# lhaippp/DMHomo

Hardware: AMD Instinct MI355X
Metric: sampled images/sec (128x128, s_step=32) (higher is better)
Workload: dtype f32; 1 GPU; DGM CFG-Unet dim=64 128x128 bs=25/GPU s_step=32 cond_scale=3 (BASELINE configs[1]); global_batch=25, cfg_mode=streams, hip_graph=True, weights=seeded random init

## Files before the change

### dmhomo_amd/_lib.py

```python
import ctypes as C
import os

import torch

_HERE = os.path.dirname(os.path.abspath(__file__))
LIB_PATH = os.environ.get('DMH_LIB_PATH') or os.path.join(_HERE, 'libdmhomo_hip.so')

c_f32p = C.c_void_p
c_i64 = C.c_int64
c_int = C.c_int
c_float = C.c_float


ABI_VERSION = 500


class DmhConv(C.Structure):
    _fields_ = [('struct_size', C.c_uint64)] + \
               [(n, C.c_void_p) for n in ('src0', 'src1', 'wpack', 'bias', 'in_coef', 'res', 'res_coef', 'out',
                                          'stats')] + \
               [(n, C.c_int32) for n in ('B', 'Hin', 'Win', 'C0', 'C1', 'Cout', 'KH', 'KW', 'stride', 'upsample2')] + \
               [('in_bound', C.c_void_p), ('in_bound_n', C.c_int32), ('fin_n', C.c_int32), ('fin_w', C.c_void_p),
                ('fin_b', C.c_void_p), ('fin_out', C.c_void_p), ('pix_stats', C.c_void_p), ('pix_eps', C.c_float),
                ('rows', C.c_void_p)]
# ... 96 lines not shown
    'dmh_linear': (c_int, [c_f32p, c_i64, c_f32p, c_f32p, c_f32p, c_i64, c_int, c_int, c_int, c_int, c_int,
                           C.c_void_p]),
    'dmh_ss_gather': (c_int, [c_f32p, c_f32p, c_f32p, C.c_void_p, C.c_void_p, C.c_void_p, c_int, c_f32p, c_int, c_int, c_int,
                              C.c_void_p]),
    'dmh_assemble_input': (c_int, [c_f32p, c_int, c_f32p, c_int, c_f32p, c_f32p, c_int, c_int, c_int, c_int,
                                   C.c_void_p]),
    'dmh_final_conv_nchw': (c_int, [c_f32p, c_f32p, c_f32p, c_f32p, c_int, c_int, c_int, c_int, C.c_void_p]),
    'dmh_sampler_step': (c_int, [C.POINTER(DmhStep), c_f32p, c_f32p, c_f32p, c_f32p, c_f32p, c_f32p, c_f32p, c_i64,
                                 C.c_void_p, c_i64, C.c_void_p]),
    'dmh_sampler_step_dev': (c_int, [C.c_void_p, c_f32p, c_f32p, c_f32p, c_f32p, c_f32p, c_f32p, c_f32p, c_i64, C.c_void_p,
                                     c_i64, C.c_void_p]),
    'dmh_sampler_seek': (c_int, [C.c_void_p, c_int, C.c_void_p, C.c_void_p, c_int, C.c_void_p, C.c_void_p, c_int,
                                 C.c_void_p]),
    'dmh_sampler_step_ddp_dev': (c_int, [C.c_void_p, C.c_void_p, C.c_void_p, c_f32p, c_f32p, c_f32p, C.c_void_p, C.c_void_p,
                                         c_f32p, c_f32p, c_int, c_int, c_int, c_int, c_int, C.c_void_p]),
    'dmh_rng_indexed': (c_int, [c_f32p, c_int, c_i64, C.c_void_p, C.c_void_p, c_int, C.c_void_p]),
    'dmh_rng_keep_mask': (c_int, [C.c_void_p, c_int, C.c_void_p, C.c_void_p, c_float, C.c_void_p]),
    'dmh_rows_lincomb': (c_int, [c_f32p, c_f32p, c_f32p, c_f32p, c_f32p, c_f32p, c_int, c_i64, c_int, C.c_void_p]),
    'dmh_pixel_grid': (c_int, [c_f32p, c_int, c_int, c_int, c_float, C.c_void_p]),
    'dmh_norm_grid': (c_int, [c_f32p, c_f32p, c_int, c_int, c_int, C.c_void_p]),
    'dmh_homography_flow_points': (c_int, [C.c_void_p, C.c_void_p, C.c_void_p, c_int, c_int, c_int, c_int, c_int, C.c_void_p]),
    'dmh_dlt_points': (c_int, [C.c_void_p, C.c_void_p, C.c_void_p, C.c_void_p, c_int, c_int, C.c_void_p]),
    'dmh_affine': (c_int, [c_f32p, c_f32p, c_float, c_float, c_i64, C.c_void_p]),
    'dmh_affine_tail': (c_int, [c_f32p, c_int, c_int, c_int, c_int, c_float, c_float, C.c_void_p]),
    'dmh_q_sample': (c_int, [c_f32p, c_f32p, c_f32p, c_f32p, c_f32p, c_int, c_i64, C.c_void_p]),
    'dmh_diff_mean': (c_int, [c_f32p, c_f32p, c_f32p, c_int, C.c_void_p, c_f32p, c_int, c_int, c_int, C.c_void_p]),
    'dmh_loss_combine': (c_int, [c_f32p, c_f32p, c_f32p, c_f32p, c_int, C.c_void_p]),
    'dmh_to_uint8': (c_int, [c_f32p, C.c_void_p, c_i64, C.c_void_p]),
    'dmh_homography_flow': (c_int, [C.c_void_p, c_f32p, c_f32p, c_int, c_int, c_int, c_float, C.c_void_p]),
    'dmh_flow_to_image': (c_int, [c_f32p, c_f32p, c_int, c_int, c_float, C.c_void_p]),
# ... 55 lines not shown
```

### dmhomo_amd/cfg.py

```python
import torch
from torch import nn

from . import _params as P
from . import ops
from ._lib import DmhStep
from .engine import UnetEngine
from .sampling import DeviceRng, ModelPrediction, ScheduleHost, default, exists, extract
from .schedule import make_buffers, ddim_pairs, linear_beta_schedule, cosine_beta_schedule


class Unet(nn.Module):

    def __init__(self, dim, num_classes, cond_drop_prob=0.5, init_dim=None, out_dim=None, dim_mults=(1, 2, 4, 8),
                 channels=3, resnet_block_groups=8, learned_variance=False, learned_sinusoidal_cond=False,
                 random_fourier_features=False, learned_sinusoidal_dim=16):
        super().__init__()
        self.cond_drop_prob = cond_drop_prob
        self.channels = channels
        input_channels = channels + 3
        init_dim = default(init_dim, dim)
        self.init_conv = nn.Conv2d(input_channels, init_dim, 7, padding=3)
        time_dim = dim * 4
        self.random_or_learned_sinusoidal_cond = learned_sinusoidal_cond or random_fourier_features
        pos_emb, fourier_dim = P.time_embedding(dim, learned_sinusoidal_cond, random_fourier_features, learned_sinusoidal_dim)
# ... 25 lines not shown
        key = (int(batch), str(torch.device(device)))
        z = cache.get(key)
        if z is None:
            z = cache[key] = torch.zeros((batch,), device=device, dtype=torch.uint8)
        return z

    def _stem(self, x, rgb_flow, mask):
        if not x.is_cuda:
            raise RuntimeError('dmhomo_amd.Unet runs on the GPU only (HIP kernels); move the inputs with .cuda()')
        eng = self._engine
        eng.ensure_prepared()
        xin = ops.assemble_input(x.to(torch.float32).contiguous(), rgb_flow.to(torch.float32).contiguous(),
                                 mask.to(torch.float32).contiguous(), reps=1, cpad=eng.cin_pad)
        return eng.stem(xin)

    def _run(self, x, time, classes, rgb_flow, mask, keeps, taps=None, x0=None, first=None, out=None, rows=None):
        eng = self._engine
        if x0 is None:
            x0 = self._stem(x, rgb_flow, mask)
        if len(keeps) > 1:
            x0 = x0.repeat(len(keeps), 1, 1, 1)
        time = time.to(torch.int64).contiguous()
        classes = classes.to(torch.int64).contiguous()
        tab = self.__dict__.get('_ss_tab')
        if tab is not None:
            T, Ct, cursor = tab
            B = classes.shape[0]
            ss_all = torch.empty((len(keeps) * B, T.shape[1]), device=T.device, dtype=torch.float32)
            for r, k in enumerate(keeps):
                ops.ss_gather(T, Ct, eng.mlp_b, cursor, classes, k, out=ss_all[r * B:(r + 1) * B])
            return eng.trunk(x0, None, taps, first=first, out=out, ss_all=ss_all, rows=rows)
        cond = eng.embed(time, [(classes, k) for k in keeps], len(keeps))
        return eng.trunk(x0, cond, taps, first=first, out=out, rows=rows)

    def forward(self, x, time, classes, rgb_flow, mask, cond_drop_prob=None):
        cond_drop_prob = default(cond_drop_prob, self.cond_drop_prob)
        keep = self._keep_mask(x.shape[0], cond_drop_prob, x.device)
        return self._run(x, time, classes, rgb_flow, mask, [keep])

    cfg_mode = 'batched'
    stream_splits = 1

    def _cond_null(self, x, time, classes, rgb_flow, mask):
        B = x.shape[0]
        keep = self._keep_mask(B, self.cond_drop_prob, x.device)
        null = self._null_mask(B, x.device)
        dedup = bool(self.dedup_dropped_rows) and keep is not None
        if self.cfg_mode == 'streams':
            nsub = max(1, min(int(self.stream_splits), B))
            nstreams = 2 * nsub
            if len(getattr(self, '_side', ())) != nstreams:
                self._side = tuple(torch.cuda.Stream(device=x.device) for _ in range(nstreams))
            cur = torch.cuda.current_stream()
            x0 = self._stem(x, rgb_flow, mask)
            first = self._engine.first_conv(x0)
            cond_out = torch.empty((B, self.out_dim) + tuple(x.shape[2:]), device=x.device, dtype=torch.float32)
            null_out = torch.empty_like(cond_out)
            bounds = [(i * B) // nsub for i in range(nsub + 1)]
            si = 0
            for k, dst, sub in ((keep, cond_out, dedup), (null, null_out, False)):
                for lo, hi in zip(bounds[:-1], bounds[1:]):
                    st = self._side[si]
                    si += 1
                    st.wait_stream(cur)
                    with torch.cuda.stream(st):
                        kk = None if k is None else k[lo:hi].contiguous()
                        fs = None if first is None else (first[0][lo:hi], first[1][lo:hi])
                        self._run(None, time[lo:hi], classes[lo:hi], None, None, [kk], x0=x0[lo:hi], first=fs, out=dst[lo:hi],
                                  rows=ops.rows_from_keep(kk) if sub else None)
            for st in self._side:
                cur.wait_stream(st)
            return cond_out, null_out, (keep if dedup else None)
        both = self._run(x, time, classes, rgb_flow, mask, [keep, null],
                         rows=ops.rows_from_keep(keep, extra=B) if dedup else None)
        return both[:B], both[B:], (keep if dedup else None)

    dedup_dropped_rows = False

    def forward_with_cond_scale(self, *args, cond_scale=1., **kwargs):
        if cond_scale == 1:
            return self.forward(*args, **kwargs)
        if 'cond_drop_prob' in kwargs or len(args) > 5:
            raise TypeError("forward() got multiple values for keyword argument 'cond_drop_prob'")
        x, time, classes, rgb_flow, mask = _bind_forward(self.forward, args, kwargs)
        logits, null, computed = self._cond_null(x, time, classes, rgb_flow, mask)
        step = DmhStep(objective=ops.OBJECTIVE['pred_x0'], clip=0, mode=ops.MODE_LAST, cond_scale=float(cond_scale),
                       sqrt_recip_ac=1., sqrt_recipm1_ac=1.)
        out, _, _ = ops.sampler_step(step, logits, null, null, None, want_x_start=False, keep=computed)
        return out
# ... 113 lines not shown
        rgb_flow = ops.affine(rgb_flow.to(torch.float32), 2., -1.)
        return self.ddim_sample(classes, rgb_flow, flow, mask, shape, cond_scale)

    def _graph_tables(self, cond_scale, clip=True):
        times, steps, draws = map(list, zip(*self._ddim_steps(clip, cond_scale)))
        return steps, times, draws

    def _sample_graphed(self, classes, rgb_flow, flow, mask, shape, cond_scale):
        m, eng, device = self.model, self.model._engine, classes.device
        clip = True
        key = (tuple(shape), tuple(rgb_flow.shape), float(cond_scale), m.cfg_mode, int(m.stream_splits),
               bool(m.dedup_dropped_rows), float(m.cond_drop_prob), self.sampling_timesteps,
               self.num_timesteps, self.objective, float(self.ddim_sampling_eta), clip, self.rng.graph_key())

        def buffers(st, times, draws):
            ins = st['ins'] = [classes.clone(), rgb_flow.to(torch.float32).clone(), mask.clone()]
            st['rf'] = torch.empty_like(ins[1])
            ops.affine(ins[1], 2., -1., out=st['rf'])
            T_tab, C_tab = eng.ss_tables(times)
            st['ss_tab'] = (T_tab, C_tab, st['cursor'])

            def mid():
                cond, null, computed = self._network(st['img'], st['tcond'], ins[0], st['rf'], ins[2], cond_scale)
                noise = self.rng.randn(shape, device).contiguous()
                ops.sampler_step_dev(st['cur'], cond, null, st['img'], noise, out=st['img'], keep=computed)
                ops.sampler_seek(st['cursor'], -1, st['table'], st['times'], st['cur'], st['tcond'])

            def last():
                cond, null, computed = self._network(st['img'], st['tcond'], ins[0], st['rf'], ins[2], cond_scale)
                x0 = ops.sampler_step_dev(st['cur'], cond, null, st['img'], None, keep=computed)
                return ops.affine(x0, 0.5, 0.5)
            return mid, last

        def fill(st):
            for dst, src in zip(st['ins'], (classes, rgb_flow, mask)):
                dst.copy_(src)
            ops.affine(st['ins'][1], 2., -1., out=st['rf'])
            st['img'].copy_(self.rng.randn(shape, device))
        img = self._replay_captured(shape, device, key, lambda: self._graph_tables(cond_scale, clip), buffers, fill)
        return img, mask, flow

    @torch.no_grad()
    def interpolate(self, x1, x2, t=None, lam=0.5):
        raise TypeError('classifier_free_guidance.GaussianDiffusion.interpolate is not callable in the reference '
                        '(CFG:733 vs CFG:639); use denoising_diffusion_pytorch.GaussianDiffusion.interpolate')

    def q_sample(self, x_start, t, noise=None):
        noise = default(noise, lambda: self.rng.randn(x_start.shape, x_start.device))
        ca = self.sqrt_alphas_cumprod.gather(-1, t).contiguous()
        cb = self.sqrt_one_minus_alphas_cumprod.gather(-1, t).contiguous()
        return ops.q_sample(x_start.contiguous(), noise.contiguous(), ca, cb)

    @property
# ... 46 lines not shown
```

### dmhomo_amd/csrc/embed.hip

```cpp
#include "common.h"

__global__ void sinusoidal_embed_kernel(const int64_t* __restrict__ t, const float* __restrict__ freq,
                                        float* __restrict__ out, int R, int dim) {
  const int idx = blockIdx.x * blockDim.x + threadIdx.x;
  const int half = dim / 2;
  if (idx >= R * half) return;
  const int r = idx / half, i = idx % half;
  const float arg = (float)t[r] * freq[i];
  out[(size_t)r * dim + i] = sinf(arg);
  out[(size_t)r * dim + half + i] = cosf(arg);
}

__global__ void fourier_embed_kernel(const int64_t* __restrict__ t, const float* __restrict__ w, float* __restrict__ out, int R,
                                     int half) {
  const int idx = blockIdx.x * blockDim.x + threadIdx.x;
  if (idx >= R * half) return;
  const int r = idx / half, i = idx % half;
  const float x = (float)t[r];
  const float arg = ((x * w[i]) * 2.0f) * 3.14159265358979323846f;
  float* o = out + (size_t)r * (2 * half + 1);
  if (i == 0) o[0] = x;
  o[1 + i] = sinf(arg);
  o[1 + half + i] = cosf(arg);
}
// ... 49 lines not shown
  if (o < out_dim && r0 + ks < R) {
    const float* q = red + (ks * 4) * 64 + ol;
    float v = (q[0] + q[64]) + (q[128] + q[192]);
    if (bias) v += bias[o];
    y[(r0 + ks) * y_stride + o] = act_f(v, act_out);
  }
}

__global__ __launch_bounds__(256) void ss_gather_kernel(const float* __restrict__ T, const float* __restrict__ Ct,
                                                        const float* __restrict__ bias, const int32_t* __restrict__ cursor,
                                                        const int64_t* __restrict__ classes, const unsigned char* __restrict__ keep,
                                                        int ncls, float* __restrict__ out, int N, int S) {
  const int b = blockIdx.y;
  const int o4 = (blockIdx.x * 256 + threadIdx.x) * 4;
  if (o4 >= N) return;
  const int step = *cursor;
  const bool kept = keep ? keep[b] != 0 : true;
  const int64_t cls = classes[b];
  if ((unsigned)step >= (unsigned)S || (kept && (cls < 0 || cls >= ncls))) {
    const float q = __builtin_nanf("");
    st4(out + (size_t)b * N + o4, make_float4(q, q, q, q));
    return;
  }
  const int row = kept ? (int)cls : ncls;
  const float4 t = ld4(T + (size_t)step * N + o4), c = ld4(Ct + (size_t)row * N + o4), bb = ld4(bias + o4);
  st4(out + (size_t)b * N + o4, make_float4((t.x + c.x) + bb.x, (t.y + c.y) + bb.y, (t.z + c.z) + bb.z, (t.w + c.w) + bb.w));
}

extern "C" int dmh_ss_gather(const float* T, const float* C, const float* bias, const int32_t* cursor, const int64_t* classes,
                             const uint8_t* keep, int ncls, float* out, int B, int N, int S, void* stream) {
  DMH_REQUIRE(T && C && bias && cursor && classes && out && B > 0 && N > 0 && N % 4 == 0 && ncls > 0 && B <= 65535 && S > 0,
              "dmh_ss_gather: bad arguments");
  hipLaunchKernelGGL(ss_gather_kernel, dim3(cdiv(N / 4, 256), B), dim3(256), 0, (hipStream_t)stream, T, C, bias, cursor, classes,
                     keep, ncls, out, N, S);
  DMH_CHECK_LAUNCH("dmh_ss_gather");
  return DMH_OK;
}

extern "C" int dmh_sinusoidal_embed(const int64_t* t, const float* freq, float* out, int R, int dim, void* stream) {
  DMH_REQUIRE(t && freq && out && R > 0 && dim > 0 && dim % 2 == 0, "dmh_sinusoidal_embed: bad arguments");
  const int total = R * (dim / 2);
// ... 34 lines not shown
```

### dmhomo_amd/csrc/philox.h

```cpp
#pragma once
#include "common.h"

#pragma clang fp contract(off)

namespace dmh_philox {

struct U4 {
  uint32_t x, y, z, w;
};

__device__ __forceinline__ U4 philox4x32_10(U4 c, uint32_t k0, uint32_t k1) {
#pragma unroll
  for (int r = 0; r < 10; ++r) {
    const uint32_t hi0 = __umulhi(0xD2511F53u, c.x), lo0 = 0xD2511F53u * c.x;
    const uint32_t hi1 = __umulhi(0xCD9E8D57u, c.z), lo1 = 0xCD9E8D57u * c.z;
    c = U4{hi1 ^ c.y ^ k0, lo1, hi0 ^ c.w ^ k1, lo0};
    k0 += 0x9E3779B9u;
    k1 += 0xBB67AE85u;
  }
  return c;
}

__device__ __forceinline__ float u01(uint32_t x) { return (float)x * 2.3283064365386963e-10f + 1.1641532182693481e-10f; }

__device__ __forceinline__ void box_muller(uint32_t a, uint32_t b, float& n0, float& n1) {
  const float r = sqrtf(-2.0f * logf(u01(a)));
  float s, c;
  sincospif(2.0f * u01(b), &s, &c);
  n0 = r * c;
  n1 = r * s;
}

__device__ __forceinline__ void normal4(uint64_t seed, uint64_t draw, uint64_t sid, uint64_t q, float v[4]) {
  const U4 r = philox4x32_10(U4{(uint32_t)q, (uint32_t)draw, (uint32_t)sid, (uint32_t)(sid >> 32)}, (uint32_t)seed,
                             (uint32_t)(seed >> 32));
  box_muller(r.x, r.y, v[0], v[1]);
  box_muller(r.z, r.w, v[2], v[3]);
}

}
```

### dmhomo_amd/csrc/rng.hip

```cpp
#include "common.h"
#include "philox.h"

#pragma clang fp contract(off)

namespace {

using namespace dmh_philox;

__global__ __launch_bounds__(256) void rng_indexed_kernel(float* __restrict__ out, int64_t per, const int64_t* __restrict__ ids,
                                                          unsigned long long* state, int kind) {
  const unsigned long long seed = state[0], draw = state[1];
  const int b = blockIdx.y;
  const unsigned long long sid = (unsigned long long)ids[b];
  float* o = out + (size_t)b * per;
  const int64_t nq = (per + 3) >> 2;
  for (int64_t q = (int64_t)blockIdx.x * 256 + threadIdx.x; q < nq; q += (int64_t)gridDim.x * 256) {
    const U4 r = philox4x32_10(U4{(uint32_t)q, (uint32_t)draw, (uint32_t)sid, (uint32_t)(sid >> 32)}, (uint32_t)seed,
                               (uint32_t)(seed >> 32));
    float v[4];
    if (kind == 0) {
      box_muller(r.x, r.y, v[0], v[1]);
      box_muller(r.z, r.w, v[2], v[3]);
    } else if (kind == 1) {
      v[0] = (float)(r.x >> 8) * 5.9604644775390625e-8f;
// ... 13 lines not shown
  __syncthreads();
  if (threadIdx.x == 0) {
    const unsigned long long total = (unsigned long long)gridDim.x * gridDim.y;
    const unsigned long long t = atomicAdd(&state[2], 1ull);
    if (t == total - 1) {
      state[2] = 0;
      state[1] = draw + 1;
    }
  }
}

__global__ __launch_bounds__(256) void rng_keep_mask_kernel(unsigned char* __restrict__ keep, int B, const int64_t* __restrict__ ids,
                                                            unsigned long long* state, float prob) {
  const unsigned long long seed = state[0], draw = state[1];
  for (int b = threadIdx.x; b < B; b += 256) {
    const unsigned long long sid = (unsigned long long)ids[b];
    const U4 r = philox4x32_10(U4{0u, (uint32_t)draw, (uint32_t)sid, (uint32_t)(sid >> 32)}, (uint32_t)seed, (uint32_t)(seed >> 32));
    keep[b] = ((float)(r.x >> 8) * 5.9604644775390625e-8f) < prob ? 1 : 0;
  }
  __syncthreads();
  if (threadIdx.x == 0) state[1] = draw + 1;
}

}

extern "C" int dmh_rng_keep_mask(uint8_t* keep, int B, const int64_t* sample_ids, uint64_t* state, float prob, void* stream) {
  DMH_REQUIRE(keep && sample_ids && state && B > 0 && B <= 65535, "dmh_rng_keep_mask: bad arguments");
  hipLaunchKernelGGL(rng_keep_mask_kernel, dim3(1), dim3(256), 0, (hipStream_t)stream, keep, B, sample_ids,
                     (unsigned long long*)state, prob);
  DMH_CHECK_LAUNCH("dmh_rng_keep_mask");
  return DMH_OK;
}

// ... 16 lines not shown
```

### dmhomo_amd/csrc/sampler.hip

```cpp
#include "common.h"
#include "philox.h"

#pragma clang fp contract(off)

__global__ __launch_bounds__(256) void assemble_input_kernel(const float* __restrict__ a, int Ca,
                                                             const float* __restrict__ b, int Cb,
                                                             const float* __restrict__ m, float* __restrict__ out,
                                                             int B, int HW, int Cpad, int64_t total) {
  for (int64_t idx = (int64_t)blockIdx.x * 256 + threadIdx.x; idx < total; idx += (int64_t)gridDim.x * 256) {
    const int c = (int)(idx % Cpad);
    const int64_t rp = idx / Cpad;
    const int p = (int)(rp % HW);
    const int r = (int)(rp / HW);
    const int s = r % B;
    float v = 0.f;
    if (c < Ca) {
      v = a[((size_t)s * Ca + c) * HW + p];
    } else if (c < Ca + Cb) {
      v = b[((size_t)s * Cb + (c - Ca)) * HW + p];
      if (m) v = v * m[(size_t)s * HW + p];
    }
    out[idx] = v;
  }
}
// ... 81 lines not shown
#pragma unroll
      for (int o = 0; o < COUT; ++o) {
        const float t = row16_sum(acc[o]);
        mine = sub == o ? t : mine;
      }
      if (sub < COUT) {
        const unsigned r = (unsigned)pix / (unsigned)HW, p = (unsigned)pix - r * (unsigned)HW;
        out[((size_t)r * COUT + sub) * HW + p] = mine + bo;
      }
    }
  }
}

__device__ __forceinline__ float clamp_pm1(float x) { return x != x ? x : fminf(fmaxf(x, -1.f), 1.f); }

__global__ __launch_bounds__(256) void sampler_step_kernel(DmhStep s, const float* __restrict__ mc,
                                                           const float* __restrict__ mn, const float* __restrict__ x,
                                                           const float* __restrict__ noise, float* __restrict__ img_out,
                                                           float* __restrict__ x_start, float* __restrict__ pred_noise,
                                                           int64_t n, const uint8_t* __restrict__ keep, int64_t per_row) {
  for (int64_t i = (int64_t)blockIdx.x * 256 + threadIdx.x; i < n; i += (int64_t)gridDim.x * 256) {
    float mo;
    if (mn) {
      const float nl = mn[i];
      mo = (keep && !keep[i / per_row]) ? nl : mc[i];
      mo = nl + (mo - nl) * s.cond_scale;
    } else {
      mo = mc[i];
    }
    const float xt = x[i];
    float x0, pn;
    if (s.objective == 0) {
      pn = mo;
      x0 = s.sqrt_recip_ac * xt - s.sqrt_recipm1_ac * pn;
      if (s.clip) x0 = clamp_pm1(x0);
    } else if (s.objective == 1) {
      x0 = mo;
      if (s.clip) x0 = clamp_pm1(x0);
      pn = (s.sqrt_recip_ac * xt - x0) / s.sqrt_recipm1_ac;
    } else {
      x0 = s.sqrt_ac * xt - s.sqrt_1m_ac * mo;
      if (s.clip) x0 = clamp_pm1(x0);
      pn = (s.sqrt_recip_ac * xt - x0) / s.sqrt_recipm1_ac;
    }
    float o;
    if (s.mode == 0) {
      o = x0 * s.c0 + s.c1 * pn + s.c2 * noise[i];
    } else if (s.mode == 1) {
      o = x0;
    } else {
      o = s.c0 * x0 + s.c1 * xt;
      if (noise) o = o + s.c2 * noise[i];
    }
    img_out[i] = o;
    if (x_start) x_start[i] = x0;
    if (pred_noise) pred_noise[i] = pn;
  }
}

__global__ __launch_bounds__(256) void sampler_step_dev_kernel(const DmhStep* __restrict__ sp, const float* __restrict__ mc,
                                                               const float* __restrict__ mn, const float* x,
                                                               const float* __restrict__ noise, float* img_out,
                                                               float* __restrict__ x_start, float* __restrict__ pred_noise,
                                                               int64_t n, const uint8_t* __restrict__ keep, int64_t per_row) {
  const DmhStep s = *sp;
  for (int64_t i = (int64_t)blockIdx.x * 256 + threadIdx.x; i < n; i += (int64_t)gridDim.x * 256) {
    float mo;
    if (mn) {
      const float nl = mn[i];
      mo = (keep && !keep[i / per_row]) ? nl : mc[i];
      mo = nl + (mo - nl) * s.cond_scale;
    } else {
      mo = mc[i];
    }
    const float xt = x[i];
    float x0, pn;
    if (s.objective == 0) {
      pn = mo;
      x0 = s.sqrt_recip_ac * xt - s.sqrt_recipm1_ac * pn;
      if (s.clip) x0 = clamp_pm1(x0);
    } else if (s.objective == 1) {
      x0 = mo;
      if (s.clip) x0 = clamp_pm1(x0);
      pn = (s.sqrt_recip_ac * xt - x0) / s.sqrt_recipm1_ac;
    } else {
      x0 = s.sqrt_ac * xt - s.sqrt_1m_ac * mo;
      if (s.clip) x0 = clamp_pm1(x0);
      pn = (s.sqrt_recip_ac * xt - x0) / s.sqrt_recipm1_ac;
    }
    float o;
    if (s.mode == 0) {
      o = x0 * s.c0 + s.c1 * pn + s.c2 * (noise ? noise[i] : __builtin_nanf(""));
    } else if (s.mode == 1) {
      o = x0;
    } else {
      o = s.c0 * x0 + s.c1 * xt;
      if (noise) o = o + s.c2 * noise[i];
    }
    img_out[i] = o;
    if (x_start) x_start[i] = x0;
    if (pred_noise) pred_noise[i] = pn;
  }
}

template <int P>
__global__ __launch_bounds__(256) void sampler_step_ddp_kernel(const DmhStep* __restrict__ sp, const int32_t* __restrict__ cursor,
                                                               const int32_t* __restrict__ draws, const float* __restrict__ mc,
                                                               float* img, const float* __restrict__ noise,
                                                               const int64_t* __restrict__ ids, unsigned long long* state,
                                                               float* __restrict__ x_start, float* __restrict__ xin, int C, int HW,
                                                               int cpad, int sc, int64_t ngroups) {
  const DmhStep s = *sp;
  const bool drawn = draws[*cursor] != 0;
// ... 32 lines not shown
      } else if (drawn && noise) {
        if constexpr (P == 4) {
          const float4 n4 = ld4(noise + base);
          nz[0] = n4.x, nz[1] = n4.y, nz[2] = n4.z, nz[3] = n4.w;
        } else {
          nz[0] = noise[base];
        }
      } else {
#pragma unroll
        for (int j = 0; j < P; ++j) nz[j] = __builtin_nanf("");
      }
#pragma unroll
      for (int j = 0; j < P; ++j) {
        const float m = mo[j], x = xt[j];
        float x0, pn;
        if (s.objective == 0) {
          pn = m;
          x0 = s.sqrt_recip_ac * x - s.sqrt_recipm1_ac * pn;
          if (s.clip) x0 = clamp_pm1(x0);
        } else if (s.objective == 1) {
          x0 = m;
          if (s.clip) x0 = clamp_pm1(x0);
          pn = (s.sqrt_recip_ac * x - x0) / s.sqrt_recipm1_ac;
        } else {
          x0 = s.sqrt_ac * x - s.sqrt_1m_ac * m;
          if (s.clip) x0 = clamp_pm1(x0);
          pn = (s.sqrt_recip_ac * x - x0) / s.sqrt_recipm1_ac;
        }
        float o;
        if (s.mode == 0) {
          o = x0 * s.c0 + s.c1 * pn + s.c2 * nz[j];
        } else if (s.mode == 1) {
          o = x0;
        } else {
          o = s.c0 * x0 + s.c1 * x;
          if (drawn) o = o + s.c2 * nz[j];
        }
        img[base + j] = o;
        if (x_start) x_start[base + j] = x0;
        if (xo) {
          if (sc) {
            xo[(size_t)j * cpad + c] = x0;
            xo[(size_t)j * cpad + C + c] = o;
          } else {
            xo[(size_t)j * cpad + c] = o;
          }
        }
      }
    }
    if (xo) {
      for (int k = cin; k < cpad; ++k)
#pragma unroll
        for (int j = 0; j < P; ++j) xo[(size_t)j * cpad + k] = 0.f;
    }
  }
  if (keyed) {
    __syncthreads();
    if (threadIdx.x == 0) {
      const unsigned long long t = atomicAdd(&state[2], 1ull);
      if (t == (unsigned long long)gridDim.x - 1) {
        state[2] = 0;
        state[1] = draw + 1;
      }
    }
  }
}

__global__ __launch_bounds__(64) void sampler_seek_kernel(int32_t* cursor, int k, const DmhStep* __restrict__ table,
                                                          const int64_t* __restrict__ times, int S, DmhStep* cur,
                                                          int64_t* tcond, int B) {
  int c = k >= 0 ? k : *cursor + 1;
  c = c < S ? c : S - 1;
  __syncthreads();
  if (threadIdx.x == 0) {
    *cursor = c;
    *cur = table[c];
  }
  const int64_t t = times[c];
  for (int i = threadIdx.x; i < B; i += 64) tcond[i] = t;
// ... 175 lines not shown
                    (((uintptr_t)model_out | (uintptr_t)img | (uintptr_t)noise | (uintptr_t)x_start) & 15) == 0;
  const int64_t ngroups = (int64_t)B * HW / (quad ? 4 : 1);
  unsigned grid = grid_for(ngroups);
  grid = grid < 1024 ? grid : 1024;
  hipStream_t st = (hipStream_t)stream;
  if (quad)
    hipLaunchKernelGGL(sampler_step_ddp_kernel<4>, dim3(grid), dim3(256), 0, st, cur_dev, cursor, draws, model_out, img, noise,
                       sample_ids, (unsigned long long*)state, x_start, xin_next, C, HW, cpad, self_cond, ngroups);
  else
    hipLaunchKernelGGL(sampler_step_ddp_kernel<1>, dim3(grid), dim3(256), 0, st, cur_dev, cursor, draws, model_out, img, noise,
                       sample_ids, (unsigned long long*)state, x_start, xin_next, C, HW, cpad, self_cond, ngroups);
  DMH_CHECK_LAUNCH("dmh_sampler_step_ddp_dev");
  return DMH_OK;
}

__global__ __launch_bounds__(64) void rows_from_keep_kernel(const uint8_t* __restrict__ keep, int B, int extra,
                                                            int32_t* __restrict__ rows) {
  int n = 0;
  for (int b0 = 0; b0 < B; b0 += 64) {
    const int b = b0 + (int)threadIdx.x;
    const bool k = b < B && keep[b] != 0;
    const unsigned long long m = __ballot(k);
    if (k) rows[1 + n + __popcll(m & ((1ull << threadIdx.x) - 1ull))] = b;
    n += __popcll(m);
  }
  for (int j = threadIdx.x; j < extra; j += 64) rows[1 + n + j] = B + j;
  if (threadIdx.x == 0) rows[0] = n + extra;
}

extern "C" int dmh_rows_from_keep(const uint8_t* keep, int B, int extra, int32_t* rows, void* stream) {
// ... 76 lines not shown
```

### dmhomo_amd/ops.py

```python
import ctypes as C

import os

import torch

from . import _lib
from ._lib import call, ptr, lib

F32 = torch.float32


def _empty(shape, like, dtype=F32):
    return torch.empty(shape, device=like.device, dtype=dtype)


def ws_standardize(w, eps=1e-5):
    w = w.detach().contiguous()
    out = torch.empty_like(w)
    cout = w.shape[0]
    call('dmh_ws_standardize', ptr(w), ptr(out), cout, w.numel() // cout, float(eps))
    return out


class PackBatch:
# ... 358 lines not shown
    cin = Cc * (2 if self_cond else 1)
    if xin is not None:
        if xin.dim() != 4 or tuple(xin.shape[:3]) != (B, H, W):
            raise ValueError(f'sampler_step_ddp_dev: xin {tuple(xin.shape)} against img {(B, Cc, H, W)}')
        cpad = xin.shape[3]
    else:
        cpad = (cin + 3) // 4 * 4
    if sample_ids is not None and sample_ids.shape[0] < B:
        raise ValueError(f'sampler_step_ddp_dev: {sample_ids.shape[0]} sample ids for {B} rows')
    call('dmh_sampler_step_ddp_dev', ptr(cur, torch.uint8), ptr(cursor, torch.int32), ptr(draws, torch.int32), ptr(model_out),
         ptr(img), ptr(noise), ptr(sample_ids, torch.int64), ptr(state, torch.int64), ptr(x_start), ptr(xin), B, Cc, H * W, cpad,
         int(bool(self_cond)))
    return img


def rng_indexed(shape, sample_ids, state, kind=0):
    B = int(shape[0])
    assert sample_ids.shape == (B,) and state.shape == (4,) and state.dtype == torch.int64
    out = torch.empty(tuple(shape), device=sample_ids.device, dtype=F32)
    call('dmh_rng_indexed', ptr(out), B, out.numel() // B, ptr(sample_ids, torch.int64), ptr(state, torch.int64), int(kind))
    return out


def rng_keep_mask(sample_ids, state, prob):
    B = sample_ids.shape[0]
    out = torch.empty((B,), device=sample_ids.device, dtype=torch.uint8)
    call('dmh_rng_keep_mask', ptr(out, torch.uint8), B, ptr(sample_ids, torch.int64), ptr(state, torch.int64), float(prob))
    return out


def affine(x, scale, shift, out=None):
    x = x.contiguous()
    y = torch.empty_like(x) if out is None else out
    call('dmh_affine', ptr(x), ptr(y), float(scale), float(shift), x.numel())
    return y


def lerp(a, b, lam):
    B = a.shape[0]
    ca = torch.full((B,), 1.0 - lam, device=a.device, dtype=torch.float32)
    cb = torch.full((B,), lam, device=a.device, dtype=torch.float32)
# ... 451 lines not shown
```

### include/dmhomo_hip.h

```cpp
#ifndef DMHOMO_HIP_H
#define DMHOMO_HIP_H

#include <stdint.h>

#ifdef __cplusplus
extern "C" {
#endif

#define DMH_OK 0
#define DMH_EINVAL (-1)
#define DMH_ELAUNCH (-2)

const char* dmh_last_error(void);
#define DMH_ABI_VERSION 500
int dmh_version(void);


int dmh_ws_standardize(const float* w, float* w_out, int Cout, int K, float eps, void* stream);

int64_t dmh_conv_pack_floats(int Cout, int C0, int C1, int KH, int KW);

int dmh_pack_conv_weight(const float* w_oihw, float* wpack, int Cout, int C0, int C1, int KH, int KW,
                         void* stream);
typedef struct DmhPackJob {
// ... 108 lines not shown
} DmhStep;
int dmh_sampler_step(const DmhStep* s, const float* model_cond, const float* model_null, const float* x,
                     const float* noise, float* img_out, float* x_start, float* pred_noise, int64_t n,
                     const uint8_t* keep, int64_t per_row, void* stream);

int dmh_sampler_step_dev(const DmhStep* cur_dev, const float* model_cond, const float* model_null, const float* x,
                         const float* noise, float* img_out, float* x_start, float* pred_noise, int64_t n,
                         const uint8_t* keep, int64_t per_row, void* stream);
int dmh_sampler_seek(int32_t* cursor, int k, const DmhStep* table, const int64_t* times, int S, DmhStep* cur,
                     int64_t* tcond, int B, void* stream);

int dmh_sampler_step_ddp_dev(const DmhStep* cur_dev, const int32_t* cursor, const int32_t* draws, const float* model_out,
                             float* img, const float* noise, const int64_t* sample_ids, uint64_t* state, float* x_start,
                             float* xin_next, int B, int C, int HW, int cpad, int self_cond, void* stream);

int dmh_rng_indexed(float* out, int B, int64_t per_sample, const int64_t* sample_ids, uint64_t* state, int kind,
                    void* stream);

int dmh_rng_keep_mask(uint8_t* keep, int B, const int64_t* sample_ids, uint64_t* state, float prob, void* stream);

int dmh_affine(const float* x, float* y, float scale, float shift, int64_t n, void* stream);
int dmh_affine_tail(float* x, int B, int C, int HW, int c0, float scale, float shift, void* stream);
int dmh_rows_lincomb(const float* x, const float* y, const float* ca, const float* cb, const float* dv, float* out, int B,
                     int64_t per_sample, int clamp, void* stream);
int dmh_q_sample(const float* x_start, const float* noise, const float* ca, const float* cb, float* out, int B,
                 int64_t per_sample, void* stream);
int dmh_diff_mean(const float* a, const float* b, const float* m, int squared, double* ws, float* out, int B, int C,
                  int HW, void* stream);
int dmh_loss_combine(const float* l, const float* photo, const float* w, float* out, int B, void* stream);
int dmh_to_uint8(const float* img, uint8_t* out, int64_t n, void* stream);
// ... 79 lines not shown
```

Measured before the change: 93.10 images/s.

## Fuse CFG sampler step with next-step input assembly, keep mask and scale-shift gather

Adds a fused device kernel for the classifier-free-guidance sampling loop. In one launch it applies the guided DDIM update, writes the next step's padded NHWC network input, redraws the keep mask, gathers the cond and null scale/shift rows, and advances the cursor and step state. The network path reuses these prepared buffers instead of re-running the stem assembly and ss_gather per stream split. This removes several small kernel launches per step inside the captured graph, in exchange for a last-block atomic handoff and a more complex state protocol.

```diff
diff --git a/dmhomo_amd/_lib.py b/dmhomo_amd/_lib.py
--- a/dmhomo_amd/_lib.py
+++ b/dmhomo_amd/_lib.py
@@ -134,6 +134,10 @@
                                  C.c_void_p]),
     'dmh_sampler_step_ddp_dev': (c_int, [C.c_void_p, C.c_void_p, C.c_void_p, c_f32p, c_f32p, c_f32p, C.c_void_p, C.c_void_p,
                                          c_f32p, c_f32p, c_int, c_int, c_int, c_int, c_int, C.c_void_p]),
+    'dmh_sampler_step_cfg_dev': (c_int, [C.c_void_p, C.c_void_p, C.c_void_p, c_int, C.c_void_p, C.c_void_p, C.c_void_p, c_f32p,
+                                         c_f32p, c_f32p, c_f32p, C.c_void_p, C.c_void_p, C.c_void_p, c_float, c_int, c_int,
+                                         c_f32p, c_f32p, c_f32p, C.c_void_p, c_int, c_f32p, c_f32p, c_int, c_int, c_int, c_int,
+                                         c_int, C.c_void_p]),
     'dmh_rng_indexed': (c_int, [c_f32p, c_int, c_i64, C.c_void_p, C.c_void_p, c_int, C.c_void_p]),
     'dmh_rng_keep_mask': (c_int, [C.c_void_p, c_int, C.c_void_p, C.c_void_p, c_float, C.c_void_p]),
     'dmh_rows_lincomb': (c_int, [c_f32p, c_f32p, c_f32p, c_f32p, c_f32p, c_f32p, c_int, c_i64, c_int, C.c_void_p]),
diff --git a/dmhomo_amd/cfg.py b/dmhomo_amd/cfg.py
--- a/dmhomo_amd/cfg.py
+++ b/dmhomo_amd/cfg.py
@@ -63,17 +63,19 @@
                                  mask.to(torch.float32).contiguous(), reps=1, cpad=eng.cin_pad)
         return eng.stem(xin)
 
-    def _run(self, x, time, classes, rgb_flow, mask, keeps, taps=None, x0=None, first=None, out=None, rows=None):
+    def _run(self, x, time, classes, rgb_flow, mask, keeps, taps=None, x0=None, first=None, out=None, rows=None, ss_all=None):
         eng = self._engine
         if x0 is None:
             x0 = self._stem(x, rgb_flow, mask)
         if len(keeps) > 1:
             x0 = x0.repeat(len(keeps), 1, 1, 1)
+        if ss_all is not None:
+            return eng.trunk(x0, None, taps, first=first, out=out, ss_all=ss_all, rows=rows)
         time = time.to(torch.int64).contiguous()
         classes = classes.to(torch.int64).contiguous()
         tab = self.__dict__.get('_ss_tab')
         if tab is not None:
-            T, Ct, cursor = tab
+            T, Ct, cursor = tab[:3]
             B = classes.shape[0]
             ss_all = torch.empty((len(keeps) * B, T.shape[1]), device=T.device, dtype=torch.float32)
             for r, k in enumerate(keeps):
@@ -92,22 +94,25 @@
 
     def _cond_null(self, x, time, classes, rgb_flow, mask):
         B = x.shape[0]
-        keep = self._keep_mask(B, self.cond_drop_prob, x.device)
+        tab = self.__dict__.get('_ss_tab')
+        prep = tab[3] if tab is not None and len(tab) > 3 else None
+        keep = prep['keep'] if prep is not None else self._keep_mask(B, self.cond_drop_prob, x.device)
         null = self._null_mask(B, x.device)
         dedup = bool(self.dedup_dropped_rows) and keep is not None
+        ss = (None, None) if prep is None else (prep['ss'][:B], prep['ss'][B:])
         if self.cfg_mode == 'streams':
             nsub = max(1, min(int(self.stream_splits), B))
             nstreams = 2 * nsub
             if len(getattr(self, '_side', ())) != nstreams:
                 self._side = tuple(torch.cuda.Stream(device=x.device) for _ in range(nstreams))
             cur = torch.cuda.current_stream()
-            x0 = self._stem(x, rgb_flow, mask)
+            x0 = self._engine.stem(prep['xin']) if prep is not None else self._stem(x, rgb_flow, mask)
             first = self._engine.first_conv(x0)
             cond_out = torch.empty((B, self.out_dim) + tuple(x.shape[2:]), device=x.device, dtype=torch.float32)
             null_out = torch.empty_like(cond_out)
             bounds = [(i * B) // nsub for i in range(nsub + 1)]
             si = 0
-            for k, dst, sub in ((keep, cond_out, dedup), (null, null_out, False)):
+            for k, dst, sub, ssp in ((keep, cond_out, dedup, ss[0]), (null, null_out, False, ss[1])):
                 for lo, hi in zip(bounds[:-1], bounds[1:]):
                     st = self._side[si]
                     si += 1
@@ -116,12 +121,12 @@
                         kk = None if k is None else k[lo:hi].contiguous()
                         fs = None if first is None else (first[0][lo:hi], first[1][lo:hi])
                         self._run(None, time[lo:hi], classes[lo:hi], None, None, [kk], x0=x0[lo:hi], first=fs, out=dst[lo:hi],
-                                  rows=ops.rows_from_keep(kk) if sub else None)
+                                  rows=ops.rows_from_keep(kk) if sub else None, ss_all=None if ssp is None else ssp[lo:hi])
             for st in self._side:
                 cur.wait_stream(st)
             return cond_out, null_out, (keep if dedup else None)
-        both = self._run(x, time, classes, rgb_flow, mask, [keep, null],
-                         rows=ops.rows_from_keep(keep, extra=B) if dedup else None)
+        both = self._run(x, time, classes, rgb_flow, mask, [keep, null], x0=None if prep is None else self._engine.stem(prep['xin']),
+                         rows=ops.rows_from_keep(keep, extra=B) if dedup else None, ss_all=None if prep is None else prep['ss'])
         return both[:B], both[B:], (keep if dedup else None)
 
     dedup_dropped_rows = False
@@ -265,11 +270,13 @@
                self.num_timesteps, self.objective, float(self.ddim_sampling_eta), clip, self.rng.graph_key())
 
         def buffers(st, times, draws):
-            ins = st['ins'] = [classes.clone(), rgb_flow.to(torch.float32).clone(), mask.clone()]
+            ins = st['ins'] = [classes.to(torch.int64).clone(), rgb_flow.to(torch.float32).clone(), mask.clone()]
             st['rf'] = torch.empty_like(ins[1])
             ops.affine(ins[1], 2., -1., out=st['rf'])
             T_tab, C_tab = eng.ss_tables(times)
             st['ss_tab'] = (T_tab, C_tab, st['cursor'])
+            if fused:
+                return fused_bodies(st, draws, T_tab, C_tab)
 
             def mid():
                 cond, null, computed = self._network(st['img'], st['tcond'], ins[0], st['rf'], ins[2], cond_scale)
@@ -283,11 +290,48 @@
                 return ops.affine(x0, 0.5, 0.5)
             return mid, last
 
+        B = int(shape[0])
+        fused = self.rng.keyed and cond_scale != 1 and (shape[2] * shape[3]) % 4 == 0
+        prob = 1 - m.cond_drop_prob
+        mask_drawn = m.cond_drop_prob > 0 and 0 < prob < 1
+
+        def fused_bodies(st, draws, T_tab, C_tab):
+            ins = st['ins']
+            st['draws'] = torch.tensor(draws, dtype=torch.int32).to(device)
+            st['xin'] = torch.zeros((B, shape[2], shape[3], eng.cin_pad), device=device)
+            st['ss'] = torch.zeros((2 * B, T_tab.shape[1]), device=device)
+            st['first'] = torch.zeros((1,), dtype=torch.int32, device=device)
+            if mask_drawn:
+                st['keep'] = torch.zeros((B,), device=device, dtype=torch.uint8)
+            else:
+                st['keep'] = m._null_mask(B, device) if m.cond_drop_prob > 0 and prob == 0 else None
+            st['ids'] = self.rng.ids_for(B)
+            st['ss_tab'] = (T_tab, C_tab, st['cursor'], {'xin': st['xin'], 'keep': st['keep'], 'ss': st['ss']})
+
+            def step():
+                cond, null, computed = self._network(st['img'], st['tcond'], ins[0], st['rf'], ins[2], cond_scale)
+                ops.sampler_step_cfg_dev(st['table'], st['times'], st['draws'], st['cursor'], st['cur'], st['tcond'], cond, null,
+                                         st['img'], st['xin'], st['ids'], self.rng.state, st['keep'],
+                                         prob if mask_drawn else None, computed is not None, T_tab, C_tab, eng.mlp_b, ins[0],
+                                         st['ss'][:B], st['ss'][B:])
+
+            def last():
+                step()
+                return ops.affine(st['img'], 0.5, 0.5)
+            return step, last
+
         def fill(st):
             for dst, src in zip(st['ins'], (classes, rgb_flow, mask)):
                 dst.copy_(src)
             ops.affine(st['ins'][1], 2., -1., out=st['rf'])
             st['img'].copy_(self.rng.randn(shape, device))
+            if 'xin' in st:
+                ins, (T_tab, C_tab) = st['ins'], st['ss_tab'][:2]
+                if mask_drawn:
+                    ops.rng_keep_mask(st['ids'], self.rng.state, prob, out=st['keep'])
+                ops.assemble_input(st['img'], st['rf'], ins[2].to(torch.float32).contiguous(), cpad=eng.cin_pad, out=st['xin'])
+                ops.ss_gather(T_tab, C_tab, eng.mlp_b, st['first'], ins[0], st['keep'], out=st['ss'][:B])
+                ops.ss_gather(T_tab, C_tab, eng.mlp_b, st['first'], ins[0], m._null_mask(B, device), out=st['ss'][B:])
         img = self._replay_captured(shape, device, key, lambda: self._graph_tables(cond_scale, clip), buffers, fill)
         return img, mask, flow
 
diff --git a/dmhomo_amd/csrc/embed.hip b/dmhomo_amd/csrc/embed.hip
--- a/dmhomo_amd/csrc/embed.hip
+++ b/dmhomo_amd/csrc/embed.hip
@@ -1,4 +1,5 @@
 #include "common.h"
+#include "ss_rows.h"
 
 __global__ void sinusoidal_embed_kernel(const int64_t* __restrict__ t, const float* __restrict__ freq,
                                         float* __restrict__ out, int R, int dim) {
@@ -87,17 +88,7 @@
   const int b = blockIdx.y;
   const int o4 = (blockIdx.x * 256 + threadIdx.x) * 4;
   if (o4 >= N) return;
-  const int step = *cursor;
-  const bool kept = keep ? keep[b] != 0 : true;
-  const int64_t cls = classes[b];
-  if ((unsigned)step >= (unsigned)S || (kept && (cls < 0 || cls >= ncls))) {
-    const float q = __builtin_nanf("");
-    st4(out + (size_t)b * N + o4, make_float4(q, q, q, q));
-    return;
-  }
-  const int row = kept ? (int)cls : ncls;
-  const float4 t = ld4(T + (size_t)step * N + o4), c = ld4(Ct + (size_t)row * N + o4), bb = ld4(bias + o4);
-  st4(out + (size_t)b * N + o4, make_float4((t.x + c.x) + bb.x, (t.y + c.y) + bb.y, (t.z + c.z) + bb.z, (t.w + c.w) + bb.w));
+  ss_row_quad(T, Ct, bias, *cursor, S, keep ? keep[b] != 0 : true, classes[b], ncls, N, o4, out + (size_t)b * N);
 }
 
 extern "C" int dmh_ss_gather(const float* T, const float* C, const float* bias, const int32_t* cursor, const int64_t* classes,
diff --git a/dmhomo_amd/csrc/philox.h b/dmhomo_amd/csrc/philox.h
--- a/dmhomo_amd/csrc/philox.h
+++ b/dmhomo_amd/csrc/philox.h
@@ -38,4 +38,9 @@
   box_muller(r.z, r.w, v[2], v[3]);
 }
 
+__device__ __forceinline__ bool keep_bit(uint64_t seed, uint64_t draw, uint64_t sid, float prob) {
+  const U4 r = philox4x32_10(U4{0u, (uint32_t)draw, (uint32_t)sid, (uint32_t)(sid >> 32)}, (uint32_t)seed, (uint32_t)(seed >> 32));
+  return ((float)(r.x >> 8) * 5.9604644775390625e-8f) < prob;
 }
+
+}
diff --git a/dmhomo_amd/csrc/rng.hip b/dmhomo_amd/csrc/rng.hip
--- a/dmhomo_amd/csrc/rng.hip
+++ b/dmhomo_amd/csrc/rng.hip
@@ -51,9 +51,7 @@
                                                             unsigned long long* state, float prob) {
   const unsigned long long seed = state[0], draw = state[1];
   for (int b = threadIdx.x; b < B; b += 256) {
-    const unsigned long long sid = (unsigned long long)ids[b];
-    const U4 r = philox4x32_10(U4{0u, (uint32_t)draw, (uint32_t)sid, (uint32_t)(sid >> 32)}, (uint32_t)seed, (uint32_t)(seed >> 32));
-    keep[b] = ((float)(r.x >> 8) * 5.9604644775390625e-8f) < prob ? 1 : 0;
+    keep[b] = keep_bit(seed, draw, (unsigned long long)ids[b], prob) ? 1 : 0;
   }
   __syncthreads();
   if (threadIdx.x == 0) state[1] = draw + 1;
diff --git a/dmhomo_amd/csrc/sampler.hip b/dmhomo_amd/csrc/sampler.hip
--- a/dmhomo_amd/csrc/sampler.hip
+++ b/dmhomo_amd/csrc/sampler.hip
@@ -1,5 +1,6 @@
 #include "common.h"
 #include "philox.h"
+#include "ss_rows.h"
 
 #pragma clang fp contract(off)
 
@@ -119,6 +120,32 @@
 
 __device__ __forceinline__ float clamp_pm1(float x) { return x != x ? x : fminf(fmaxf(x, -1.f), 1.f); }
 
+__device__ __forceinline__ float step_guided(const DmhStep& s, float cond, float nl) { return nl + (cond - nl) * s.cond_scale; }
+
+__device__ __forceinline__ void step_predict(const DmhStep& s, float mo, float xt, float& x0, float& pn) {
+  if (s.objective == 0) {
+    pn = mo;
+    x0 = s.sqrt_recip_ac * xt - s.sqrt_recipm1_ac * pn;
+    if (s.clip) x0 = clamp_pm1(x0);
+  } else if (s.objective == 1) {
+    x0 = mo;
+    if (s.clip) x0 = clamp_pm1(x0);
+    pn = (s.sqrt_recip_ac * xt - x0) / s.sqrt_recipm1_ac;
+  } else {
+    x0 = s.sqrt_ac * xt - s.sqrt_1m_ac * mo;
+    if (s.clip) x0 = clamp_pm1(x0);
+    pn = (s.sqrt_recip_ac * xt - x0) / s.sqrt_recipm1_ac;
+  }
+}
+
+__device__ __forceinline__ float step_update(const DmhStep& s, float x0, float pn, float xt, float nz, bool has_nz) {
+  if (s.mode == 0) return x0 * s.c0 + s.c1 * pn + s.c2 * nz;
+  if (s.mode == 1) return x0;
+  float o = s.c0 * x0 + s.c1 * xt;
+  if (has_nz) o = o + s.c2 * nz;
+  return o;
+}
+
 __global__ __launch_bounds__(256) void sampler_step_kernel(DmhStep s, const float* __restrict__ mc,
                                                            const float* __restrict__ mn, const float* __restrict__ x,
                                                            const float* __restrict__ noise, float* __restrict__ img_out,
@@ -128,35 +155,14 @@
     float mo;
     if (mn) {
       const float nl = mn[i];
-      mo = (keep && !keep[i / per_row]) ? nl : mc[i];
-      mo = nl + (mo - nl) * s.cond_scale;
+      mo = step_guided(s, (keep && !keep[i / per_row]) ? nl : mc[i], nl);
     } else {
       mo = mc[i];
     }
     const float xt = x[i];
     float x0, pn;
-    if (s.objective == 0) {
-      pn = mo;
-      x0 = s.sqrt_recip_ac * xt - s.sqrt_recipm1_ac * pn;
-      if (s.clip) x0 = clamp_pm1(x0);
-    } else if (s.objective == 1) {
-      x0 = mo;
-      if (s.clip) x0 = clamp_pm1(x0);
-      pn = (s.sqrt_recip_ac * xt - x0) / s.sqrt_recipm1_ac;
-    } else {
-      x0 = s.sqrt_ac * xt - s.sqrt_1m_ac * mo;
-      if (s.clip) x0 = clamp_pm1(x0);
-      pn = (s.sqrt_recip_ac * xt - x0) / s.sqrt_recipm1_ac;
-    }
-    float o;
-    if (s.mode == 0) {
-      o = x0 * s.c0 + s.c1 * pn + s.c2 * noise[i];
-    } else if (s.mode == 1) {
-      o = x0;
-    } else {
-      o = s.c0 * x0 + s.c1 * xt;
-      if (noise) o = o + s.c2 * noise[i];
-    }
+    step_predict(s, mo, xt, x0, pn);
+    const float o = step_update(s, x0, pn, xt, noise ? noise[i] : __builtin_nanf(""), noise != nullptr);
     img_out[i] = o;
     if (x_start) x_start[i] = x0;
     if (pred_noise) pred_noise[i] = pn;
@@ -173,35 +179,14 @@
     float mo;
     if (mn) {
       const float nl = mn[i];
-      mo = (keep && !keep[i / per_row]) ? nl : mc[i];
-      mo = nl + (mo - nl) * s.cond_scale;
+      mo = step_guided(s, (keep && !keep[i / per_row]) ? nl : mc[i], nl);
     } else {
       mo = mc[i];
     }
     const float xt = x[i];
     float x0, pn;
-    if (s.objective == 0) {
-      pn = mo;
-      x0 = s.sqrt_recip_ac * xt - s.sqrt_recipm1_ac * pn;
-      if (s.clip) x0 = clamp_pm1(x0);
-    } else if (s.objective == 1) {
-      x0 = mo;
-      if (s.clip) x0 = clamp_pm1(x0);
-      pn = (s.sqrt_recip_ac * xt - x0) / s.sqrt_recipm1_ac;
-    } else {
-      x0 = s.sqrt_ac * xt - s.sqrt_1m_ac * mo;
-      if (s.clip) x0 = clamp_pm1(x0);
-      pn = (s.sqrt_recip_ac * xt - x0) / s.sqrt_recipm1_ac;
-    }
-    float o;
-    if (s.mode == 0) {
-      o = x0 * s.c0 + s.c1 * pn + s.c2 * (noise ? noise[i] : __builtin_nanf(""));
-    } else if (s.mode == 1) {
-      o = x0;
-    } else {
-      o = s.c0 * x0 + s.c1 * xt;
-      if (noise) o = o + s.c2 * noise[i];
-    }
+    step_predict(s, mo, xt, x0, pn);
+    const float o = step_update(s, x0, pn, xt, noise ? noise[i] : __builtin_nanf(""), noise != nullptr);
     img_out[i] = o;
     if (x_start) x_start[i] = x0;
     if (pred_noise) pred_noise[i] = pn;
@@ -264,28 +249,8 @@
       for (int j = 0; j < P; ++j) {
         const float m = mo[j], x = xt[j];
         float x0, pn;
-        if (s.objective == 0) {
-          pn = m;
-          x0 = s.sqrt_recip_ac * x - s.sqrt_recipm1_ac * pn;
-          if (s.clip) x0 = clamp_pm1(x0);
-        } else if (s.objective == 1) {
-          x0 = m;
-          if (s.clip) x0 = clamp_pm1(x0);
-          pn = (s.sqrt_recip_ac * x - x0) / s.sqrt_recipm1_ac;
-        } else {
-          x0 = s.sqrt_ac * x - s.sqrt_1m_ac * m;
-          if (s.clip) x0 = clamp_pm1(x0);
-          pn = (s.sqrt_recip_ac * x - x0) / s.sqrt_recipm1_ac;
-        }
-        float o;
-        if (s.mode == 0) {
-          o = x0 * s.c0 + s.c1 * pn + s.c2 * nz[j];
-        } else if (s.mode == 1) {
-          o = x0;
-        } else {
-          o = s.c0 * x0 + s.c1 * x;
-          if (drawn) o = o + s.c2 * nz[j];
-        }
+        step_predict(s, m, x, x0, pn);
+        const float o = step_update(s, x0, pn, x, nz[j], drawn);
         img[base + j] = o;
         if (x_start) x_start[base + j] = x0;
         if (xo) {
@@ -313,6 +278,122 @@
         state[1] = draw + 1;
       }
     }
+  }
+}
+
+struct CfgStepArgs {
+  const DmhStep* table;
+  const int64_t* times;
+  const int32_t* draws;
+  int S;
+  int32_t* cursor;
+  DmhStep* cur;
+  int64_t* tcond;
+  const float* mc;
+  const float* mn;
+  float* img;
+  float* xin;
+  const int64_t* ids;
+  unsigned long long* state;
+  uint8_t* keep;
+  float prob;
+  int draw_mask, dedup;
+  const float* T;
+  const float* Ct;
+  const float* bias;
+  const int64_t* classes;
+  int ncls;
+  float* ss_cond;
+  float* ss_null;
+  int N, B, C, HW, cpad;
+  int64_t ngroups;
+};
+
+template <int CT>
+__global__ __launch_bounds__(256) void sampler_step_cfg_kernel(const CfgStepArgs a) {
+  using namespace dmh_philox;
+  const DmhStep s = *a.cur;
+  const int k = *a.cursor;
+  const bool drawn = (unsigned)k < (unsigned)a.S && a.draws[k] != 0;
+  const unsigned long long seed = a.state[0], draw = a.state[1];
+  const int C = CT > 0 ? CT : a.C;
+  const int HW = a.HW, G = HW >> 2;
+  for (int64_t g = (int64_t)blockIdx.x * 256 + threadIdx.x; g < a.ngroups; g += (int64_t)gridDim.x * 256) {
+    const int b = (int)(g / G);
+    const int p0 = (int)(g - (int64_t)b * G) * 4;
+    const bool kept = !a.dedup || a.keep[b] != 0;
+    const unsigned long long sid = drawn ? (unsigned long long)a.ids[b] : 0ull;
+    float* xo = a.xin + ((size_t)b * HW + p0) * a.cpad;
+    constexpr int NQ = CT > 0 ? CT : 1;
+    float oq[NQ][4];
+#pragma unroll NQ
+    for (int c = 0; c < C; ++c) {
+      const size_t base = ((size_t)b * C + c) * HW + p0;
+      const float4 n4 = ld4(a.mn + base), x4 = ld4(a.img + base);
+      const float4 c4 = kept ? ld4(a.mc + base) : n4;
+      const float cd[4] = {c4.x, c4.y, c4.z, c4.w}, nl[4] = {n4.x, n4.y, n4.z, n4.w}, xt[4] = {x4.x, x4.y, x4.z, x4.w};
+      float nz[4], o[4];
+      if (drawn) {
+        normal4(seed, draw, sid, (uint64_t)(((int64_t)c * HW + p0) >> 2), nz);
+      } else {
+#pragma unroll
+        for (int j = 0; j < 4; ++j) nz[j] = __builtin_nanf("");
+      }
+#pragma unroll
+      for (int j = 0; j < 4; ++j) {
+        float x0, pn;
+        step_predict(s, step_guided(s, cd[j], nl[j]), xt[j], x0, pn);
+        o[j] = step_update(s, x0, pn, xt[j], nz[j], drawn);
+      }
+      st4(a.img + base, make_float4(o[0], o[1], o[2], o[3]));
+      if (drawn) {
+#pragma unroll
+        for (int j = 0; j < 4; ++j) {
+          if constexpr (CT > 0) oq[c][j] = o[j];
+          else xo[(size_t)j * a.cpad + c] = o[j];
+        }
+      }
+    }
+    if constexpr (CT > 0) {
+      if (drawn) {
+#pragma unroll
+        for (int j = 0; j < 4; ++j) {
+          float* px = xo + (size_t)j * a.cpad;
+#pragma unroll
+          for (int q = 0; q + 4 <= CT; q += 4) st4(px + q, make_float4(oq[q][j], oq[q + 1][j], oq[q + 2][j], oq[q + 3][j]));
+#pragma unroll
+          for (int c = CT & ~3; c < CT; ++c) px[c] = oq[c][j];
+        }
+      }
+    }
+  }
+  if (!drawn) return;
+  const int kn = k + 1 < a.S ? k + 1 : a.S - 1;
+  const int N4 = a.N >> 2;
+  const int64_t items = (int64_t)2 * a.B * N4;
+  for (int64_t i = (int64_t)blockIdx.x * 256 + threadIdx.x; i < items; i += (int64_t)gridDim.x * 256) {
+    const int r = (int)(i / N4), o4 = (int)(i - (int64_t)r * N4) * 4;
+    const bool null_pass = r >= a.B;
+    const int b = null_pass ? r - a.B : r;
+    bool kept = false;
+    if (!null_pass)
+      kept = a.draw_mask ? keep_bit(seed, draw + 1, (unsigned long long)a.ids[b], a.prob) : (a.keep ? a.keep[b] != 0 : true);
+    ss_row_quad(a.T, a.Ct, a.bias, kn, a.S, kept, a.classes[b], a.ncls, a.N, o4, (null_pass ? a.ss_null : a.ss_cond) + (size_t)b * a.N);
+  }
+  __shared__ int last;
+  __syncthreads();
+  if (threadIdx.x == 0) last = atomicAdd(&a.state[2], 1ull) == (unsigned long long)gridDim.x - 1;
+  __syncthreads();
+  if (!last) return;
+  if (a.draw_mask)
+    for (int b = threadIdx.x; b < a.B; b += 256) a.keep[b] = keep_bit(seed, draw + 1, (unsigned long long)a.ids[b], a.prob) ? 1 : 0;
+  const int64_t tn = a.times[kn];
+  for (int i = threadIdx.x; i < a.B; i += 256) a.tcond[i] = tn;
+  if (threadIdx.x == 0) {
+    a.state[2] = 0;
+    a.state[1] = draw + (a.draw_mask ? 2ull : 1ull);
+    *a.cursor = kn;
+    *a.cur = a.table[kn];
   }
 }
 
@@ -518,6 +599,44 @@
   return DMH_OK;
 }
 
+extern "C" int dmh_sampler_step_cfg_dev(const DmhStep* table, const int64_t* times, const int32_t* draws, int S, int32_t* cursor,
+                                        DmhStep* cur, int64_t* tcond, const float* model_cond, const float* model_null,
+                                        float* img, float* xin_next, const int64_t* sample_ids, uint64_t* state, uint8_t* keep,
+                                        float keep_prob, int draw_mask, int dedup, const float* T, const float* Ct,
+                                        const float* bias, const int64_t* classes, int ncls, float* ss_cond, float* ss_null,
+                                        int N, int B, int C, int HW, int cpad, void* stream) {
+  DMH_REQUIRE(table && times && draws && cursor && cur && tcond && S > 0, "dmh_sampler_step_cfg_dev: step tables / cursor missing");
+  DMH_REQUIRE(model_cond && model_null && img && xin_next && sample_ids && state && B > 0 && C > 0 && HW > 0,
+              "dmh_sampler_step_cfg_dev: bad arguments");
+  DMH_REQUIRE(T && Ct && bias && classes && ss_cond && ss_null && ncls > 0 && N > 0 && N % 4 == 0 && (int64_t)B * N < ((int64_t)1 << 30),
+              "dmh_sampler_step_cfg_dev: (scale, shift) tables: N=%d must be a positive multiple of 4, B*N < 2^30", N);
+  DMH_REQUIRE((draw_mask == 0 || draw_mask == 1) && (dedup == 0 || dedup == 1) && (!draw_mask || keep) && (!dedup || keep),
+              "dmh_sampler_step_cfg_dev: draw_mask / dedup need the keep buffer");
+  DMH_REQUIRE(C <= 4096 && cpad % 4 == 0 && cpad >= C && cpad <= 16384,
+              "dmh_sampler_step_cfg_dev: cpad=%d must be a multiple of 4 >= %d channels", cpad, C);
+  DMH_REQUIRE(HW % 4 == 0 && (int64_t)B * HW < ((int64_t)1 << 31) && (int64_t)C * HW < ((int64_t)1 << 34),
+              "dmh_sampler_step_cfg_dev: HW=%d must be a multiple of 4, B*HW < 2^31, C*HW < 2^34", HW);
+  DMH_REQUIRE((((uintptr_t)model_cond | (uintptr_t)model_null | (uintptr_t)img | (uintptr_t)xin_next | (uintptr_t)T | (uintptr_t)Ct |
+                (uintptr_t)bias | (uintptr_t)ss_cond | (uintptr_t)ss_null) & 15) == 0,
+              "dmh_sampler_step_cfg_dev: tensors must be 16-byte aligned");
+  CfgStepArgs a;
+  a.table = table, a.times = times, a.draws = draws, a.S = S, a.cursor = cursor, a.cur = cur, a.tcond = tcond;
+  a.mc = model_cond, a.mn = model_null, a.img = img, a.xin = xin_next;
+  a.ids = sample_ids, a.state = (unsigned long long*)state, a.keep = keep, a.prob = keep_prob, a.draw_mask = draw_mask, a.dedup = dedup;
+  a.T = T, a.Ct = Ct, a.bias = bias, a.classes = classes, a.ncls = ncls, a.ss_cond = ss_cond, a.ss_null = ss_null;
+  a.N = N, a.B = B, a.C = C, a.HW = HW, a.cpad = cpad;
+  a.ngroups = (int64_t)B * HW / 4;
+  unsigned grid = grid_for(a.ngroups);
+  grid = grid < 512 ? grid : 512;
+  hipStream_t st = (hipStream_t)stream;
+  if (C == 6)
+    hipLaunchKernelGGL(sampler_step_cfg_kernel<6>, dim3(grid), dim3(256), 0, st, a);
+  else
+    hipLaunchKernelGGL(sampler_step_cfg_kernel<0>, dim3(grid), dim3(256), 0, st, a);
+  DMH_CHECK_LAUNCH("dmh_sampler_step_cfg_dev");
+  return DMH_OK;
+}
+
 __global__ __launch_bounds__(64) void rows_from_keep_kernel(const uint8_t* __restrict__ keep, int B, int extra,
                                                             int32_t* __restrict__ rows) {
   int n = 0;
diff --git a/dmhomo_amd/csrc/ss_rows.h b/dmhomo_amd/csrc/ss_rows.h
--- /dev/null
+++ b/dmhomo_amd/csrc/ss_rows.h
@@ -0,0 +1,15 @@
+#pragma once
+#include "common.h"
+
+__device__ __forceinline__ void ss_row_quad(const float* __restrict__ T, const float* __restrict__ Ct,
+                                            const float* __restrict__ bias, int step, int S, bool kept, int64_t cls, int ncls,
+                                            int N, int o4, float* __restrict__ row) {
+  if ((unsigned)step >= (unsigned)S || (kept && (cls < 0 || cls >= ncls))) {
+    const float q = __builtin_nanf("");
+    st4(row + o4, make_float4(q, q, q, q));
+    return;
+  }
+  const int r = kept ? (int)cls : ncls;
+  const float4 t = ld4(T + (size_t)step * N + o4), c = ld4(Ct + (size_t)r * N + o4), bb = ld4(bias + o4);
+  st4(row + o4, make_float4((t.x + c.x) + bb.x, (t.y + c.y) + bb.y, (t.z + c.z) + bb.z, (t.w + c.w) + bb.w));
+}
diff --git a/dmhomo_amd/ops.py b/dmhomo_amd/ops.py
--- a/dmhomo_amd/ops.py
+++ b/dmhomo_amd/ops.py
@@ -396,6 +396,29 @@
     return img
 
 
+def sampler_step_cfg_dev(table, times, draws, cursor, cur, tcond, model_cond, model_null, img, xin, sample_ids, state, keep,
+                         keep_prob, dedup, T, Ct, bias, classes, ss_cond, ss_null):
+    B, Cc, H, W = img.shape
+    N = T.shape[1]
+    for t in (model_cond, model_null):
+        if tuple(t.shape) != (B, Cc, H, W):
+            raise ValueError(f'sampler_step_cfg_dev: {tuple(t.shape)} against img {(B, Cc, H, W)}')
+    if xin.dim() != 4 or tuple(xin.shape[:3]) != (B, H, W):
+        raise ValueError(f'sampler_step_cfg_dev: xin {tuple(xin.shape)} against img {(B, Cc, H, W)}')
+    if tuple(ss_cond.shape) != (B, N) or tuple(ss_null.shape) != (B, N) or Ct.shape[1] != N or bias.shape != (N,):
+        raise ValueError(f'sampler_step_cfg_dev: (scale, shift) rows {tuple(ss_cond.shape)} / {tuple(ss_null.shape)} against {(B, N)}')
+    if sample_ids.shape[0] < B or classes.shape[0] != B or tcond.shape[0] != B or (keep is not None and keep.shape[0] != B):
+        raise ValueError(f'sampler_step_cfg_dev: per-row vectors against {B} rows')
+    if draws.shape[0] != times.shape[0]:
+        raise ValueError(f'sampler_step_cfg_dev: {draws.shape[0]} draw flags for {times.shape[0]} steps')
+    call('dmh_sampler_step_cfg_dev', ptr(table, torch.uint8), ptr(times, torch.int64), ptr(draws, torch.int32), times.shape[0],
+         ptr(cursor, torch.int32), ptr(cur, torch.uint8), ptr(tcond, torch.int64), ptr(model_cond), ptr(model_null), ptr(img),
+         ptr(xin), ptr(sample_ids, torch.int64), ptr(state, torch.int64), ptr(keep, torch.uint8),
+         float(keep_prob if keep_prob is not None else 0.), int(keep_prob is not None), int(bool(dedup)), ptr(T), ptr(Ct),
+         ptr(bias), ptr(classes, torch.int64), Ct.shape[0] - 1, ptr(ss_cond), ptr(ss_null), N, B, Cc, H * W, xin.shape[3])
+    return img
+
+
 def rng_indexed(shape, sample_ids, state, kind=0):
     B = int(shape[0])
     assert sample_ids.shape == (B,) and state.shape == (4,) and state.dtype == torch.int64
@@ -404,9 +427,11 @@
     return out
 
 
-def rng_keep_mask(sample_ids, state, prob):
+def rng_keep_mask(sample_ids, state, prob, out=None):
     B = sample_ids.shape[0]
-    out = torch.empty((B,), device=sample_ids.device, dtype=torch.uint8)
+    if out is None:
+        out = torch.empty((B,), device=sample_ids.device, dtype=torch.uint8)
+    assert out.shape == (B,)
     call('dmh_rng_keep_mask', ptr(out, torch.uint8), B, ptr(sample_ids, torch.int64), ptr(state, torch.int64), float(prob))
     return out
 
diff --git a/include/dmhomo_hip.h b/include/dmhomo_hip.h
--- a/include/dmhomo_hip.h
+++ b/include/dmhomo_hip.h
@@ -146,6 +146,13 @@
                              float* img, const float* noise, const int64_t* sample_ids, uint64_t* state, float* x_start,
                              float* xin_next, int B, int C, int HW, int cpad, int self_cond, void* stream);
 
+int dmh_sampler_step_cfg_dev(const DmhStep* table, const int64_t* times, const int32_t* draws, int S, int32_t* cursor,
+                             DmhStep* cur, int64_t* tcond, const float* model_cond, const float* model_null, float* img,
+                             float* xin_next, const int64_t* sample_ids, uint64_t* state, uint8_t* keep, float keep_prob,
+                             int draw_mask, int dedup, const float* T, const float* Ct, const float* bias,
+                             const int64_t* classes, int ncls, float* ss_cond, float* ss_null, int N, int B, int C, int HW,
+                             int cpad, void* stream);
+
 int dmh_rng_indexed(float* out, int B, int64_t per_sample, const int64_t* sample_ids, uint64_t* state, int kind,
                     void* stream);
 
```

After: 93.63 images/s, median of 6. Within noise of the previous version (+0.6%).
